# arnab39/equiadapt

Hardware: AMD Instinct MI355X
Metric: canonicalize+invert images/sec (224x224 C8) (higher is better)
Workload: dtype f32 (resampling / FFT / accumulation in fp32; the network's channel contraction as 2xfp16 split of every fp32 operand (within one fp32 ulp), 3 exact products, fp32 accumulate -- closer to fp64 than the fp32 matrix instruction, see step_ms_by_gemm_form); 1 GPU; configs[1]: 224x224x3 synthetic, C8, GroupEquivariantImageCanonicalization + ESCNNEquivariantNetwork in e2cnn's LAYER SHAPES (32 fields x 8 = 256 ch, k5, 3 layers, crop 0.8, resize 96) with this repository's own filter-bank parameterisation (bilinear-rotated banks; e2cnn's steerable basis is not restated -- e2cnn-trained weights enter via load_exported_dense), forward, then invert_canonicalization; batch_per_gpu=256, global_batch=256, parallelism=dp1 (no collective in the forward path)

## Files before the change

### equiadapt_amd/csrc/lift_fft.hip

```cpp
#include <cstdlib>

#include "eqa_common.hpp"

#ifndef EQA_LF_AUX
#define EQA_LF_AUX 2
#endif

namespace {

#include "fft_common.inc"

typedef float f32x4 __attribute__((ext_vector_type(4)));
typedef unsigned u32x4 __attribute__((ext_vector_type(4)));

#ifdef EQA_LF_CLOCK
__device__ unsigned long long g_lf_clock[32];
#define LF_CLOCK_BEGIN() const bool lfc_on = blockIdx.x == 0 && (threadIdx.x & 63) == 0 && (wave == 0 || wave == 1 || wave == 8); \
  unsigned long long lfc_t = __builtin_readcyclecounter(); unsigned long long lfc_s[16] = {0, 0, 0, 0, 0, 0, 0, 0, 0, 0, 0, 0, 0, 0, 0, 0}
#define LF_CLOCK(i) do { const unsigned long long n_ = __builtin_readcyclecounter(); lfc_s[i] += n_ - lfc_t; lfc_t = n_; } while (0)
#define LF_CLOCK_END() do { if (lfc_on) for (int i_ = 0; i_ < 8; ++i_) g_lf_clock[8 * (ROLE == kConv ? 0 : (wave == 1 ? 1 : 2)) + i_] = lfc_s[i_]; } while (0)
#else
#define LF_CLOCK_BEGIN() do { } while (0)
#define LF_CLOCK(i) do { } while (0)
#define LF_CLOCK_END() do { } while (0)
#endif

constexpr int kLfThreads = 768;
constexpr int kLfCh = 16;
constexpr int kLfSteps = 19;
constexpr int kLfQuadPitch = 196;
constexpr int kLfRowPitch = 784;
constexpr int kLfTileFloats = kFftN * kLfRowPitch;
constexpr int kLfSubRows = 16;
constexpr int kLfPatchRows = kLfSubRows + 4, kLfPatchPitch = 156;
constexpr int kLfPatchFloats = kLfPatchRows * kLfPatchPitch;
constexpr int kLfLdsFloats = kLfTileFloats + kLfPatchFloats;
constexpr int kLfStagers = 6 * 64;
constexpr int kLfPre = (kLfPatchFloats + kLfStagers - 1) / kLfStagers;

__device__ __forceinline__ void lf_slot(int n, int& ky, int& e, bool& spare) {
  spare = n == 75;
  const bool lo = n < 70;
  const int r = n % 14;
  ky = lo ? n / 14 : min(n - 70, 4);
  e = lo ? (r >> 1) + 8 * (r & 1) : 7;
}

struct LfItem {
  unsigned grp, m;
  int gy0, gx0;
  size_t img;
};

__device__ __forceinline__ LfItem lf_item(unsigned work, int ngrp, int TY, int TX) {
  LfItem it;
  it.grp = work % ngrp;
#ifdef EQA_LF_XCDGRP
  if (ngrp == 16) it.grp = 2 * (it.grp % 8) + it.grp / 8;
#endif
  it.m = work / ngrp;
  const unsigned tx = it.m % TX, ty = (it.m / TX) % TY;
  it.img = it.m / ((unsigned)TX * TY);
  it.gy0 = kFftO * (int)ty;
  it.gx0 = kFftO * (int)tx;
  return it;
}

enum { kConv = 0, kCols = 1, kRowp = 2 };

template <class F, int... Is>
__device__ __forceinline__ void lf_for_const(F&& f, std::integer_sequence<int, Is...>) {
  (f(std::integral_constant<int, Is>()), ...);
}

constexpr int kLpRowB = 53 * 8;
constexpr int kLpPlaneB = 8 * kLpRowB;
constexpr int kLpPatchB = 3 * kLpPlaneB;
constexpr int kLpLdsBytes = kLfTileFloats * 4 + kLpPatchB;
constexpr int kLhRowB = 52 * 8;
constexpr int kLhRing = 16;
constexpr int kLhPlaneB = kLhRing * kLhRowB;
constexpr int kLhPatchB = 2 * kLhPlaneB;
constexpr int kLhLdsBytes = kLfTileFloats * 4 + kLhPatchB;
constexpr int kLhSubRows = 12;
constexpr int kLhPre = 3;
typedef _Float16 lf_f16x8 __attribute__((ext_vector_type(8)));
typedef _Float16 lf_f16x4 __attribute__((ext_vector_type(4)));
typedef __bf16 lf_bf16x8 __attribute__((ext_vector_type(8)));
typedef __bf16 lf_bf16x4 __attribute__((ext_vector_type(4)));
__device__ __forceinline__ void lf_split3(float x, __bf16& p1, __bf16& p2, __bf16& p3) {
  p1 = (__bf16)x;
  const float r1 = x - (float)p1;
  p2 = (__bf16)r1;
  p3 = (__bf16)(r1 - (float)p2);
}

template <int ROLE, int FORM>
__device__ __forceinline__ void lift5_fft48_body(const float* __restrict__ x, const float* __restrict__ bank, const float* __restrict__ bias,
                                                 int relu, float* __restrict__ V, int H0, int W0, int C, int TY, int TX, size_t Mp,
                                                 unsigned nwork, unsigned v_bytes, unsigned x_bytes, unsigned bank_bytes,
                                                 float* __restrict__ dcmax, const float* __restrict__ xbound, int nxbound, float w_scale) {
  constexpr bool COLS = ROLE == kCols;
  constexpr bool PIECES = FORM == 3;
  constexpr bool H2 = FORM == 2;
  constexpr int NSUB = PIECES ? 12 : (H2 ? 4 : 3);
  constexpr int SUBROWS = kFftN / NSUB;
  constexpr int NGRP = 12 / NSUB;
  extern __shared__ float lds[];
  float* const tile = lds;
  float* const patch = lds + kLfTileFloats;
  const int tid = threadIdx.x;
  const int lane = tid & 63;
  const int wave = __builtin_amdgcn_readfirstlane(tid >> 6);
  const int j = lane & 15, q = lane >> 4;
  const int ngrp = C / kLfCh;
  const int H1 = H0 - 4, W1 = W0 - 4;
  const unsigned nblk = gridDim.x;
  const unsigned patch_b = (unsigned)(kLfTileFloats * 4);
  LF_CLOCK_BEGIN();

  const __amdgpu_buffer_rsrc_t xr = __builtin_amdgcn_make_buffer_rsrc(const_cast<float*>(x), 0, x_bytes, 0x00020000);
  float pre[COLS ? kLfPre : 1];
  auto prefetch = [&](const LfItem& it, int sub, bool live) {
    if constexpr (COLS) {
      int tq = tid;
      asm volatile("" : "+v"(tq));
#pragma unroll
      for (int i = 0; i < kLfPre; ++i) {
        const int idx = tq + kLfStagers * i;
        const int pr = idx / kLfPatchPitch, pc = idx - pr * kLfPatchPitch;
        const int gy = it.gy0 + kLfSubRows * sub + pr, gxc = it.gx0 * 3 + pc;
        const bool ok = live && idx < kLfPatchFloats && gy < H0 && gxc < W0 * 3;
        const unsigned off = ok ? (unsigned)(((it.img * H0 + gy) * (size_t)(W0 * 3) + gxc) * 4) : 0xfffffff0u;
        pre[i] = __builtin_bit_cast(float, __builtin_amdgcn_raw_buffer_load_b32(xr, off, 0, 0));
      }
    }
  };
  auto stage = [&]() {
    if constexpr (COLS) {
#pragma unroll
      for (int i = 0; i < kLfPre; ++i) {
        const int idx = tid + kLfStagers * i;
        if (idx < kLfPatchFloats) patch[idx] = pre[i];
      }
    }
  };

  float preg[COLS && PIECES ? 2 : 1][3];
  auto prefetch_grp = [&](const LfItem& it, int g, int which, bool live) {
    if constexpr (COLS && PIECES) {
      int tq = tid;
      asm volatile("" : "+v"(tq));
      const int pr = tq / 52, px = tq - pr * 52;
      const int gy = it.gy0 + 4 * g + pr, gx = it.gx0 + px;
      const bool ok = live && tq < 208 && gy < H0 && gx < W0;
      const unsigned off = ok ? (unsigned)((((it.img * H0 + gy) * (size_t)W0 + gx) * 3) * 4) : 0xfffffff0u;
#pragma unroll
      for (int c = 0; c < 3; ++c) preg[which][c] = __builtin_bit_cast(float, __builtin_amdgcn_raw_buffer_load_b32(xr, off, c * 4, 0));
    }
  };
  auto stage_grp = [&](int g, int which) {
    if constexpr (COLS && PIECES) {
      if (tid < 208) {
        const int pr = tid / 52, px = tid - pr * 52;
        __bf16 pc[3][3];
#pragma unroll
        for (int c = 0; c < 3; ++c) lf_split3(preg[which][c], pc[0][c], pc[1][c], pc[2][c]);
        char* dst = reinterpret_cast<char*>(lds) + patch_b + ((4 * g + pr) & 7) * kLpRowB + px * 8;
#pragma unroll
        for (int pl = 0; pl < 3; ++pl) {
          const lf_bf16x4 v = {pc[pl][0], pc[pl][1], pc[pl][2], (__bf16)0.0f};
          *reinterpret_cast<lf_bf16x4*>(dst + pl * kLpPlaneB) = v;
        }
      }
    }
  };

  float preh[(!COLS && H2) ? kLhPre : 1][3];
  float x_scale = 1.0f, out_scale = 1.0f;
  if constexpr (H2) {
    float mx = 0.0f;
    for (int t = lane; t < nxbound; t += 64) mx = fmaxf(mx, xbound[t]);
#pragma unroll
    for (int o = 32; o > 0; o >>= 1) mx = fmaxf(mx, __shfl_xor(mx, o));
    int ex = 0;
    if (mx > 0.0f && mx < 3.0e38f) (void)frexpf(mx, &ex);
    ex = __builtin_amdgcn_readfirstlane(min(max(14 - ex, -100), 100));
    x_scale = ldexpf(1.0f, ex);
    out_scale = ldexpf(1.0f, -ex) / w_scale;
  }
  int h_pr[(!COLS && H2) ? kLhPre : 1], h_px[(!COLS && H2) ? kLhPre : 1];
  if constexpr (!COLS && H2) {
#pragma unroll
    for (int i = 0; i < kLhPre; ++i) {
      const int idx = tid - 6 * 64 + kLfStagers * i;
      h_pr[i] = idx / 52;
      h_px[i] = idx - h_pr[i] * 52;
    }
  }
  auto prefetch_h = [&](const LfItem& it, int row0, int nrows, bool live) {
    if constexpr (!COLS && H2) {
#ifdef EQA_LF_H2_NOPREFETCH
      if (row0 >= 0) return;
#endif
#pragma unroll
      for (int i = 0; i < kLhPre; ++i) {
        const int pr = h_pr[i], px = h_px[i];
        const int gy = it.gy0 + row0 + pr, gx = it.gx0 + px;
        const bool ok = live && pr < nrows && gy < H0 && gx < W0;
        const unsigned off = ok ? (unsigned)((((it.img * H0 + gy) * (size_t)W0 + gx) * 3) * 4) : 0xfffffff0u;
#pragma unroll
        for (int c = 0; c < 3; ++c) preh[i][c] = __builtin_bit_cast(float, __builtin_amdgcn_raw_buffer_load_b32(xr, off, c * 4, 0));
      }
    }
  };
  auto stage_h = [&](int row0, int nrows) {
    if constexpr (!COLS && H2) {
#pragma unroll
      for (int i = 0; i < kLhPre; ++i) {
        asm volatile("" : "+v"(preh[i][0]), "+v"(preh[i][1]), "+v"(preh[i][2]));
        if (h_pr[i] < nrows) {
          const int pr = h_pr[i], px = h_px[i];
          _Float16 hi[3], lo[3];
#pragma unroll
          for (int c = 0; c < 3; ++c) {
            const float v = preh[i][c] * x_scale;
            hi[c] = (_Float16)v;
            lo[c] = (_Float16)(v - (float)hi[c]);
          }
          char* dst = reinterpret_cast<char*>(lds) + patch_b + ((row0 + pr) & (kLhRing - 1)) * kLhRowB + px * 8;
          const lf_f16x4 vh = {hi[0], hi[1], hi[2], (_Float16)0.0f}, vl = {lo[0], lo[1], lo[2], (_Float16)0.0f};
          *reinterpret_cast<lf_f16x4*>(dst) = vh;
          *reinterpret_cast<lf_f16x4*>(dst + kLhPlaneB) = vl;
        }
      }
    }
  };

  const int nr = (wave == 10 || wave == 11) ? 2 : 3;
  const int r0 = wave == 8 ? 0 : (wave == 9 ? 3 : (wave == 6 ? 6 : (wave == 10 ? 9 : (wave == 7 ? 11 : 14))));
  unsigned a_off[kLfSteps];
  float wreg[kLfSteps];
  f32x4 bias4;
  auto setup = [&](const LfItem& it) {
    const __amdgpu_buffer_rsrc_t br = __builtin_amdgcn_make_buffer_rsrc(const_cast<float*>(bank), 0, bank_bytes, 0x00020000);
    const unsigned wb = (unsigned)((it.grp * kLfCh + j) * 75 * 4);
#pragma unroll
    for (int t = 0; t < kLfSteps; ++t) {
      int ky, e;
      bool spare;
      lf_slot(4 * t + q, ky, e, spare);
      a_off[t] = patch_b + (unsigned)(((r0 + ky) * kLfPatchPitch + j * 3 + e) * 4);
      wreg[t] = __builtin_bit_cast(float, __builtin_amdgcn_raw_buffer_load_b32(br, spare ? 0xfffffff0u : wb + (unsigned)((ky * 15 + e) * 4), 0, 0));
    }
#pragma unroll
    for (int r = 0; r < 4; ++r) bias4[r] = bias ? bias[it.grp * kLfCh + 4 * q + r] : 0.0f;
    asm volatile("" : "+v"(bias4));
  };
#ifndef EQA_LF_AHEAD
#define EQA_LF_AHEAD 5
#endif
  constexpr int kAhead = EQA_LF_AHEAD;
  auto conv_rows = [&](const LfItem& it, int y0) {
    float b[3][kLfSteps], bq[2][3][kAhead];
    auto lds_at = [&](int t, int drow, int tx3) {
#ifdef EQA_LF_NOLDSREAD
      return __builtin_bit_cast(float, a_off[t] + (unsigned)(drow + tx3));
#else
      return reinterpret_cast<const float*>(reinterpret_cast<const char*>(lds) + a_off[t])[drow * kLfPatchPitch + tx3 * 48];
#endif
    };
#pragma unroll
    for (int t = 0; t < kAhead; ++t)
#pragma unroll
      for (int tx3 = 0; tx3 < 3; ++tx3) bq[0][tx3][t] = lds_at(t, 0, tx3);
#pragma unroll
    for (int r = 0; r < 3; ++r) {
      if (r < nr) {
        const int par = r & 1;
        const bool row_ok = it.gy0 + y0 + r < H1;
        f32x4 acc[3] = {bias4, bias4, bias4};
        __builtin_amdgcn_sched_barrier(0);
#pragma unroll
        for (int t = 0; t < kLfSteps; ++t) {
#pragma unroll
          for (int tx3 = 0; tx3 < 3; ++tx3)
#ifdef EQA_LF_NOMFMA
            acc[tx3][t & 3] += wreg[t] * (t < kAhead ? bq[par][tx3][t] : b[tx3][t]);
#else
            acc[tx3] = __builtin_amdgcn_mfma_f32_16x16x4f32(wreg[t], t < kAhead ? bq[par][tx3][t] : b[tx3][t], acc[tx3], 0, 0, 0);
#endif
          __builtin_amdgcn_sched_barrier(0);
          if (t + kAhead < kLfSteps) {
#pragma unroll
            for (int tx3 = 0; tx3 < 3; ++tx3) b[tx3][t + kAhead] = lds_at(t + kAhead, r, tx3);
          } else if (r + 1 < nr) {
#pragma unroll
            for (int tx3 = 0; tx3 < 3; ++tx3) bq[par ^ 1][tx3][t + kAhead - kLfSteps] = lds_at(t + kAhead - kLfSteps, r + 1, tx3);
          }
          __builtin_amdgcn_sched_barrier(0);
        }
#pragma unroll
        for (int tx3 = 0; tx3 < 3; ++tx3) {
          const bool ok = row_ok && it.gx0 + tx3 * 16 + j < W1;
          f32x4 v = acc[tx3];
#pragma unroll
          for (int k = 0; k < 4; ++k) {
            float u = relu ? fmaxf(v[k], 0.0f) : v[k];
            v[k] = ok ? u : 0.0f;
          }
          *reinterpret_cast<f32x4*>(tile + (y0 + r) * kLfRowPitch + q * kLfQuadPitch + (tx3 * 16 + j) * 4) = v;
        }
      }
    }
  };

  lf_bf16x8 wq[PIECES ? 4 : 1][PIECES ? 3 : 1];
  unsigned c_off[PIECES ? 4 : 1];
  int c_ky[PIECES ? 4 : 1];
  auto setup_p = [&](const LfItem& it) {
    if constexpr (PIECES) {
      const __amdgpu_buffer_rsrc_t br = __builtin_amdgcn_make_buffer_rsrc(const_cast<float*>(bank), 0, bank_bytes, 0x00020000);
#pragma unroll
      for (int sstep = 0; sstep < 4; ++sstep) {
        const int c = 4 * sstep + q;
        c_ky[sstep] = min(c / 3, 4);
        c_off[sstep] = (unsigned)((j + 2 * (c % 3)) * 8);
#pragma unroll
        for (int wp = 0; wp < 3; ++wp) {
          const unsigned off = (unsigned)((((it.grp * kLfCh + j) * 3 + wp) * 16 + c) * 16);
          wq[sstep][wp] = __builtin_bit_cast(lf_bf16x8, __builtin_amdgcn_raw_buffer_load_b128(br, off, 0, 0));
        }
      }
#pragma unroll
      for (int r = 0; r < 4; ++r) bias4[r] = bias ? bias[it.grp * kLfCh + 4 * q + r] : 0.0f;
      asm volatile("" : "+v"(bias4));
    }
  };
  auto conv_tiles_p = [&](const LfItem& it, int y, int tx0, auto NT) {
    constexpr int nt = decltype(NT)::value;
    if constexpr (PIECES) {
      const bool row_ok = it.gy0 + y < H1;
      unsigned addr[4];
#pragma unroll
      for (int sstep = 0; sstep < 4; ++sstep) addr[sstep] = patch_b + (unsigned)(((y + c_ky[sstep]) & 7) * kLpRowB) + c_off[sstep] + (unsigned)(tx0 * 16 * 8);
      f32x4 acc[3] = {bias4, bias4, bias4};
      lf_bf16x8 bp[2][3][3];
      auto read_step = [&](int sstep, int buf) {
#pragma unroll
        for (int t = 0; t < 3; ++t)
          if (t < nt)
#pragma unroll
            for (int pl = 0; pl < 3; ++pl)
#ifdef EQA_LF_NOLDSREAD
            {
              const f32x4 cv = {1.0f + (float)(addr[sstep] & 7), 0.5f + t, 0.25f + pl, 2.0f};
              bp[buf][t][pl] = __builtin_bit_cast(lf_bf16x8, cv);
            }
#else
            {
              typedef unsigned long long u64x2_t __attribute__((ext_vector_type(2)));
              const unsigned long long* pp = reinterpret_cast<const unsigned long long*>(reinterpret_cast<const char*>(lds) + addr[sstep] + t * 128 + pl * kLpPlaneB);
              const u64x2_t two = {pp[0], pp[1]};
              bp[buf][t][pl] = __builtin_bit_cast(lf_bf16x8, two);
            }
#endif
      };
      read_step(0, 0);
#pragma unroll
      for (int sstep = 0; sstep < 4; ++sstep) {
        const int buf = sstep & 1;
        if (sstep + 1 < 4) read_step(sstep + 1, buf ^ 1);
        __builtin_amdgcn_sched_barrier(0);
        constexpr int kW[6] = {2, 0, 1, 1, 0, 0}, kP[6] = {0, 2, 1, 0, 1, 0};
#pragma unroll
        for (int pr = 0; pr < 6; ++pr) {
#pragma unroll
          for (int t = 0; t < 3; ++t)
            if (t < nt) acc[t] = __builtin_amdgcn_mfma_f32_16x16x32_bf16(wq[sstep][kW[pr]], bp[buf][t][kP[pr]], acc[t], 0, 0, 0);
          __builtin_amdgcn_sched_barrier(0);
        }
      }
#pragma unroll
      for (int t = 0; t < 3; ++t) {
        if (t < nt) {
          const int tx3 = tx0 + t;
          const bool ok = row_ok && it.gx0 + tx3 * 16 + j < W1;
          f32x4 v = acc[t];
#pragma unroll
          for (int k = 0; k < 4; ++k) {
            float u = relu ? fmaxf(v[k], 0.0f) : v[k];
            v[k] = ok ? u : 0.0f;
          }
          *reinterpret_cast<f32x4*>(tile + y * kLfRowPitch + q * kLfQuadPitch + (tx3 * 16 + j) * 4) = v;
        }
      }
    }
  };

  lf_f16x8 wh[H2 ? 5 : 1][H2 ? 2 : 1];
  int h_off = 0;
  auto setup_h = [&](const LfItem& it) {
    if constexpr (H2) {
      const __amdgpu_buffer_rsrc_t br = __builtin_amdgcn_make_buffer_rsrc(const_cast<float*>(bank), 0, bank_bytes, 0x00020000);
#pragma unroll
      for (int ky = 0; ky < 5; ++ky)
#pragma unroll
        for (int wp = 0; wp < 2; ++wp) {
          const unsigned off = (unsigned)(((((it.grp * kLfCh + j) * 2 + wp) * 5 + ky) * 4 + q) * 16);
          wh[ky][wp] = __builtin_bit_cast(lf_f16x8, __builtin_amdgcn_raw_buffer_load_b128(br, off, 0, 0));
        }
#pragma unroll
      for (int r = 0; r < 4; ++r) bias4[r] = bias ? bias[it.grp * kLfCh + 4 * q + r] : 0.0f;
      asm volatile("" : "+v"(bias4));
    }
  };
  auto conv_col_h = [&](const LfItem& it, int y0, int t, auto NR) {
    if constexpr (H2) {
      constexpr int NROWS = decltype(NR)::value;
#ifdef EQA_LF_H2_NOCONV
      return;
#endif
      const int base = (int)patch_b + (j - 1 + 2 * min(q, 2)) * 8 + t * 128;
      lf_f16x8 win[7][2];
      auto read_row = [&](int k) {
        const int a = base + ((y0 + k) & (kLhRing - 1)) * kLhRowB;
#pragma unroll
        for (int pl = 0; pl < 2; ++pl) {
          typedef unsigned long long u64x2_t __attribute__((ext_vector_type(2)));
          const unsigned long long* pp = reinterpret_cast<const unsigned long long*>(reinterpret_cast<const char*>(lds) + a + pl * kLhPlaneB);
          const u64x2_t two = {pp[0], pp[1]};
          win[k % 7][pl] = __builtin_bit_cast(lf_f16x8, two);
        }
      };
#pragma unroll
      for (int k = 0; k < 6; ++k) read_row(k);
      const f32x4 zero = {0.0f, 0.0f, 0.0f, 0.0f};
      const bool col_ok = it.gx0 + t * 16 + j < W1;
      f32x4 acc[2];
      f32x4 ev = zero;
      auto epi = [&](int m, int rp) {
        const int y = y0 + rp;
        if (m == 0) ev = acc[rp & 1] * out_scale + bias4;
        else if (m == 1) { ev[0] = relu ? fmaxf(ev[0], 0.0f) : ev[0]; ev[1] = relu ? fmaxf(ev[1], 0.0f) : ev[1]; }
        else if (m == 2) { ev[2] = relu ? fmaxf(ev[2], 0.0f) : ev[2]; ev[3] = relu ? fmaxf(ev[3], 0.0f) : ev[3]; }
        else if (m == 3) {
          const bool ok = col_ok && it.gy0 + y < H1;
#pragma unroll
          for (int k = 0; k < 4; ++k) ev[k] = ok ? ev[k] : 0.0f;
        } else if (m == 4) {
          *reinterpret_cast<f32x4*>(tile + y * kLfRowPitch + q * kLfQuadPitch + (t * 16 + j) * 4) = ev;
        }
      };
#pragma unroll
      for (int r = 0; r < NROWS; ++r) {
#pragma unroll
        for (int m = 0; m < 15; ++m) {
          const int ky = m / 3, ch = m % 3;
          __builtin_amdgcn_sched_barrier(0);
          acc[r & 1] = __builtin_amdgcn_mfma_f32_16x16x32_f16(wh[ky][ch == 0 ? 1 : 0], win[(r + ky) % 7][ch == 1 ? 1 : 0], m == 0 ? zero : acc[r & 1], 0, 0, 0);
          if (r > 0 && m >= 2 && m < 7) epi(m - 2, r - 1);
          if (m == 9 && r + 2 < NROWS) read_row(r + 6);
        }
      }
      __builtin_amdgcn_sched_barrier(0);
#pragma unroll
      for (int m = 0; m < 5; ++m) epi(m, NROWS - 1);
    }
  };

  auto row_pass = [&](int y0) {
#ifdef EQA_LF_H2_NOROWP
    if (H2) return;
#endif
    float* const rowp = tile + (y0 + (lane >> 4)) * kLfRowPitch + ((lane & 15) >> 2) * kLfQuadPitch + (lane & 3);
    float re[kFftN], ore[kFftH], oim[kFftH];
#pragma unroll
    for (int xx = 0; xx < kFftN; ++xx) re[xx] = rowp[xx * 4];
    fft48_r2c(re, ore, oim);
#pragma unroll
    for (int k = 0; k < kFftH - 1; ++k) rowp[k * 4] = ore[k];
    rowp[24 * 4] = ore[24];
#pragma unroll
    for (int k = 1; k < kFftH - 1; ++k) rowp[(24 + k) * 4] = oim[k];
  };

  const int cw = COLS ? wave : 0;
  const int col_ci = lane >> 4, col_kxi = (lane >> 2) & 3, col_cq = lane & 3;
  const int kc_of0 = 8 * (cw >> 1) + 2 * (cw & 1) + (col_kxi >> 1);
  const int kc = kc_of0 + ((col_kxi & 1) ? 4 : 0);
  const bool odd = (col_kxi & 1) != 0;
  const bool has_packed = COLS && __builtin_amdgcn_readfirstlane((int)(cw == 0)) != 0;
  const bool pair_packed = COLS && kc_of0 == 0;
  const bool packed = COLS && kc == 0;
  const float* const colp = tile + col_cq * kLfQuadPitch + col_ci + kc * 4;
  const __amdgpu_buffer_rsrc_t vr = __builtin_amdgcn_make_buffer_rsrc(V, 0, v_bytes, 0x00020000);
  float cre[kFftN], cim[kFftN];
  unsigned pend_m = 0, pend_grp = 0;
  bool pending = false;
  float dc_seen = 0.0f;
  auto transpose4 = [&](float& r0_, float& r1_, float& r2_, float& r3_) {
    auto sw16 = [](float& a, float& b) { asm volatile("s_nop 1\n\tv_permlane16_swap_b32 %0, %1" : "+v"(a), "+v"(b)); };
    auto sw32 = [](float& a, float& b) { asm volatile("s_nop 1\n\tv_permlane32_swap_b32 %0, %1" : "+v"(a), "+v"(b)); };
    sw16(r0_, r1_);
    sw16(r2_, r3_);
    sw32(r0_, r2_);
    sw32(r1_, r3_);
  };
  auto swz4 = [](float v) { return __builtin_bit_cast(float, __builtin_amdgcn_ds_swizzle(__builtin_bit_cast(int, v), 0x101f)); };
  auto store_pair = [&](float* re, float* im, unsigned voff1, unsigned voff2, bool second) {
    transpose4(re[0], re[1], re[2], re[3]);
    transpose4(im[0], im[1], im[2], im[3]);
    f32x4 o1, o2;
#pragma unroll
    for (int r = 0; r < 4; ++r) {
      const float got = swz4(odd ? re[r] : im[r]);
      o1[r] = odd ? got : re[r];
      o2[r] = odd ? im[r] : got;
    }
    __builtin_amdgcn_raw_buffer_store_b128(__builtin_bit_cast(u32x4, o1), vr, voff1, 0, EQA_LF_AUX);
    if (second) __builtin_amdgcn_raw_buffer_store_b128(__builtin_bit_cast(u32x4, o2), vr, voff2, 0, EQA_LF_AUX);
  };
  auto col_work = [&](auto SUB) {
    constexpr int sub = decltype(SUB)::value;
    if (!pending) return;
#ifdef EQA_LF_H2_NOCOLS
    if (H2) return;
#endif
    const size_t rowb = Mp * 2 * (size_t)C * 4;
    const unsigned col = (unsigned)(((size_t)pend_m * 2 * C + pend_grp * 2 * kLfCh) * 4) + (unsigned)((odd ? 64 : 0) + 16 * col_cq);
    if (sub == 0) {
      float ore[kFftN], oim[kFftN];
      fft48(cre, cim, ore, oim);
#pragma unroll
      for (int ky = 0; ky < kFftN; ++ky) {
        cre[ky] = ore[ky];
        cim[ky] = oim[ky];
      }
      if (has_packed) {
        float p24re[28], p24im[28];
#pragma unroll
        for (int ky = 0; ky < kFftH; ++ky) {
          const int kn = (kFftN - ky) % kFftN;
          const float a = ore[ky], b = oim[ky], c2 = ore[kn], d = oim[kn];
          p24re[ky] = 0.5f * (b + d);
          p24im[ky] = 0.5f * (c2 - a);
          cre[ky] = packed ? 0.5f * (a + c2) : a;
          cim[ky] = packed ? 0.5f * (b - d) : b;
        }
        dc_seen = fmaxf(dc_seen, packed ? cre[0] : 0.0f);
#pragma unroll
        for (int ky = kFftH; ky < 28; ++ky) p24re[ky] = p24im[ky] = 0.0f;
#ifndef EQA_LF_NOSTORE
        const unsigned vb24 = (unsigned)((size_t)(kFftN * kFftInner + 1 + 2 * col_ci) * rowb) + col;
#pragma unroll
        for (int g = 0; g < 7; ++g) {
          const bool live = pair_packed && 4 * g + col_ci < kFftH;
          store_pair(&p24re[4 * g], &p24im[4 * g], live ? vb24 + (unsigned)g * (unsigned)(8 * rowb) : 0xfffffff0u, 0xfffffff0u, false);
        }
#endif
      }
    }
#ifndef EQA_LF_NOSTORE
    const unsigned f1 = pair_packed ? (unsigned)(kFftN * kFftInner + 2 * col_ci) : (unsigned)(kFftInner * col_ci + kc_of0 - 1);
    const unsigned vb1 = (unsigned)((size_t)f1 * rowb) + col, vs1 = (unsigned)((pair_packed ? 8 : 4 * kFftInner) * rowb);
    const unsigned vb2 = (unsigned)((size_t)(kFftInner * col_ci + kc_of0 + 3) * rowb) + col, vs2 = (unsigned)(4 * kFftInner * rowb);
#pragma unroll
    for (int g = NGRP * sub; g < NGRP * sub + NGRP; ++g) {
      const bool live1 = !pair_packed || 4 * g + col_ci < kFftH;
      store_pair(&cre[4 * g], &cim[4 * g], live1 ? vb1 + (unsigned)g * vs1 : 0xfffffff0u, vb2 + (unsigned)g * vs2, true);
    }
#endif
  };

  unsigned cur_grp = 0xffffffffu;
  unsigned v = blockIdx.x;
  if constexpr (PIECES) {
    if (COLS && tid < 24) *reinterpret_cast<unsigned long long*>(reinterpret_cast<char*>(lds) + patch_b + tid * kLpRowB + 52 * 8) = 0ull;
    const LfItem f = lf_item(v < nwork ? v : 0, ngrp, TY, TX);
    prefetch_grp(f, 0, 0, v < nwork);
    prefetch_grp(f, 1, 1, v < nwork);
    stage_grp(0, 0);
    stage_grp(1, 1);
  } else if constexpr (H2) {
    if (tid == 0) *reinterpret_cast<unsigned long long*>(reinterpret_cast<char*>(lds) + patch_b - 8) = 0ull;
    prefetch_h(lf_item(v < nwork ? v : 0, ngrp, TY, TX), 0, kLhRing, v < nwork);
    stage_h(0, kLhRing);
    __syncthreads();
  } else {
    if (v < nwork) prefetch(lf_item(v, ngrp, TY, TX), 0, true);
    stage();
    __syncthreads();
  }
  for (;; v += nblk) {
    const bool live = v < nwork;
    if (!live && !pending) break;
    const LfItem it = lf_item(live ? v : 0, ngrp, TY, TX);
    const unsigned vn = v + nblk;
    const bool next_live = live && vn < nwork;
    const LfItem nx = lf_item(next_live ? vn : 0, ngrp, TY, TX);
    if constexpr (!COLS) {
#pragma unroll 1
      for (int sub = 0; sub < NSUB; ++sub) {
        if (PIECES || sub > 0) __syncthreads();
        LF_CLOCK(0);
        if constexpr (H2) {
          if (sub < NSUB - 1) prefetch_h(it, kLhSubRows * sub + kLhRing, kLhSubRows, live);
          else prefetch_h(nx, 0, kLhRing, next_live);
          LF_CLOCK(1);
        }
        if (live) {
          if (sub == 0 && it.grp != cur_grp) {
            if constexpr (PIECES) setup_p(it);
            else if constexpr (H2) { if constexpr (ROLE == kConv) setup_h(it); }
            else setup(it);
            cur_grp = it.grp;
          }
          if constexpr (H2) {
            if constexpr (ROLE == kConv) {
              conv_col_h(it, kLhSubRows * sub, wave - 8, std::integral_constant<int, kLhSubRows>());
            } else {
              if (sub > 0) row_pass(kLhSubRows * (sub - 1) + 4 * (wave == 11 ? 2 : wave - 6));
            }
          } else if constexpr (PIECES) {
            const int y = SUBROWS * sub + (wave == 8 ? 0 : (wave == 9 ? 1 : ((wave == 6 || wave == 10) ? 2 : 3)));
            const int tx0 = (wave == 10 || wave == 11) ? 2 : 0;
            if (wave == 8 || wave == 9) conv_tiles_p(it, y, tx0, std::integral_constant<int, 3>());
            else if (wave == 10 || wave == 11) conv_tiles_p(it, y, tx0, std::integral_constant<int, 1>());
            else conv_tiles_p(it, y, tx0, std::integral_constant<int, 2>());
          } else {
            conv_rows(it, kLfSubRows * sub + r0);
            if (sub > 0 && (wave == 8 || wave == 9)) row_pass(8 * (sub - 1) + 4 * (wave - 8));
          }
        }
        LF_CLOCK(2);
        __syncthreads();
        LF_CLOCK(3);
        if constexpr (H2) {
          if (sub < NSUB - 1) stage_h(kLhSubRows * sub + kLhRing, kLhSubRows);
          else stage_h(0, kLhRing);
        }
      }
    } else {
      auto subphase = [&](auto SUB) {
        constexpr int sub = decltype(SUB)::value;
        if constexpr (FORM == 0) {
          if (sub > 0) stage();
        }
        if (PIECES || sub > 0) __syncthreads();
        LF_CLOCK(0);
        if constexpr (H2) {
        } else if constexpr (PIECES) {
          if (sub < NSUB - 1) {
            prefetch_grp(it, sub + 2, 0, live);
          } else {
            prefetch_grp(nx, 0, 0, next_live);
            prefetch_grp(nx, 1, 1, next_live);
          }
        } else {
          if (sub < NSUB - 1) prefetch(it, sub + 1, live);
          else prefetch(nx, 0, next_live);
        }
        LF_CLOCK(1);
        col_work(SUB);
        LF_CLOCK(2);
        __syncthreads();
        LF_CLOCK(3);
        if constexpr (PIECES) {
          if (sub < NSUB - 1) {
            stage_grp(sub + 2, 0);
          } else {
            stage_grp(0, 0);
            stage_grp(1, 1);
          }
        }
      };
      lf_for_const(subphase, std::make_integer_sequence<int, NSUB>());
      if constexpr (FORM == 0) stage();
    }
    if constexpr (PIECES) {
      if (live) row_pass(4 * wave);
    } else if constexpr (H2) {
      if constexpr (ROLE == kRowp) {
        if (live) row_pass(36 + 4 * (wave == 11 ? 2 : wave - 6));
      }
    } else {
      if (live && wave < 8) row_pass(16 + 4 * wave);
    }
    LF_CLOCK(4);
    __syncthreads();
    LF_CLOCK(5);
    constexpr int kEarly = PIECES ? kFftN : (H2 ? kLhSubRows : kLfSubRows);
    if constexpr (COLS) {
      if (live) {
#pragma unroll
        for (int y = 0; y < kEarly; ++y) {
          cre[y] = colp[y * kLfRowPitch];
          cim[y] = colp[y * kLfRowPitch + 24 * 4];
        }
      }
    }
    LF_CLOCK(6);
    __syncthreads();
    LF_CLOCK(7);
    if constexpr (COLS && !PIECES) {
      if (live) {
#pragma unroll
        for (int y = kEarly; y < kFftN; ++y) {
          cre[y] = colp[y * kLfRowPitch];
          cim[y] = colp[y * kLfRowPitch + 24 * 4];
        }
      }
    }
    pend_m = it.m;
    pend_grp = it.grp;
    pending = live;
  }
  if constexpr (COLS) {
    if (dcmax != nullptr && has_packed) {
      float m = dc_seen;
#pragma unroll
      for (int o = 32; o > 0; o >>= 1) m = fmaxf(m, __shfl_xor(m, o));
      if (lane == 0) dcmax[blockIdx.x] = m;
      if (blockIdx.x == 0) {
        for (unsigned t = nblk + lane; t < (unsigned)EQA_LIFT5_DCMAX_SLOTS; t += 64) dcmax[t] = 0.0f;
      }
    }
  }
  LF_CLOCK_END();
}

__global__ __launch_bounds__(kLfThreads) void lift5_fft48_fused_kernel(const float* __restrict__ x, const float* __restrict__ bank,
                                                                        const float* __restrict__ bias, int relu, float* __restrict__ V,
                                                                        int H0, int W0, int C, int TY, int TX, size_t Mp, unsigned nwork,
                                                                        unsigned v_bytes, unsigned x_bytes, unsigned bank_bytes,
                                                                        float* __restrict__ dcmax) {
  if (threadIdx.x < 6 * 64) lift5_fft48_body<kCols, 0>(x, bank, bias, relu, V, H0, W0, C, TY, TX, Mp, nwork, v_bytes, x_bytes, bank_bytes, dcmax, nullptr, 0, 1.0f);
  else lift5_fft48_body<kConv, 0>(x, bank, bias, relu, V, H0, W0, C, TY, TX, Mp, nwork, v_bytes, x_bytes, bank_bytes, dcmax, nullptr, 0, 1.0f);
}

__global__ __launch_bounds__(kLfThreads) void lift5_fft48_fused_pieces_kernel(const float* __restrict__ x, const float* __restrict__ bank,
                                                                               const float* __restrict__ bias, int relu, float* __restrict__ V,
                                                                               int H0, int W0, int C, int TY, int TX, size_t Mp, unsigned nwork,
                                                                               unsigned v_bytes, unsigned x_bytes, unsigned bank_bytes,
                                                                               float* __restrict__ dcmax) {
  if (threadIdx.x < 6 * 64) lift5_fft48_body<kCols, 3>(x, bank, bias, relu, V, H0, W0, C, TY, TX, Mp, nwork, v_bytes, x_bytes, bank_bytes, dcmax, nullptr, 0, 1.0f);
  else lift5_fft48_body<kConv, 3>(x, bank, bias, relu, V, H0, W0, C, TY, TX, Mp, nwork, v_bytes, x_bytes, bank_bytes, dcmax, nullptr, 0, 1.0f);
}

__global__ __launch_bounds__(kLfThreads) void lift5_fft48_fused_h2_kernel(const float* __restrict__ x, const float* __restrict__ bank,
                                                                           const float* __restrict__ bias, int relu, float* __restrict__ V,
                                                                           int H0, int W0, int C, int TY, int TX, size_t Mp, unsigned nwork,
                                                                           unsigned v_bytes, unsigned x_bytes, unsigned bank_bytes,
                                                                           float* __restrict__ dcmax, const float* __restrict__ xbound,
                                                                           int nxbound, float w_scale) {
  const int w = __builtin_amdgcn_readfirstlane((int)(threadIdx.x >> 6));
  if (w < 6) lift5_fft48_body<kCols, 2>(x, bank, bias, relu, V, H0, W0, C, TY, TX, Mp, nwork, v_bytes, x_bytes, bank_bytes, dcmax, xbound, nxbound, w_scale);
  else if (w >= 8 && w <= 10) lift5_fft48_body<kConv, 2>(x, bank, bias, relu, V, H0, W0, C, TY, TX, Mp, nwork, v_bytes, x_bytes, bank_bytes, dcmax, xbound, nxbound, w_scale);
  else lift5_fft48_body<kRowp, 2>(x, bank, bias, relu, V, H0, W0, C, TY, TX, Mp, nwork, v_bytes, x_bytes, bank_bytes, dcmax, xbound, nxbound, w_scale);
}

__global__ __launch_bounds__(256) void absmax_slots_kernel(const float* __restrict__ x, size_t n, float* __restrict__ out) {
  float m = 0.0f;
  const size_t n4 = n / 4;
  for (size_t i = (size_t)blockIdx.x * 256 + threadIdx.x; i < n4; i += (size_t)gridDim.x * 256) {
    const f32x4 v = reinterpret_cast<const f32x4*>(x)[i];
    m = fmaxf(fmaxf(m, fmaxf(fabsf(v[0]), fabsf(v[1]))), fmaxf(fabsf(v[2]), fabsf(v[3])));
  }
  if (blockIdx.x == 0 && threadIdx.x < (n & 3)) m = fmaxf(m, fabsf(x[n4 * 4 + threadIdx.x]));
  __shared__ float red[4];
#pragma unroll
  for (int o = 32; o > 0; o >>= 1) m = fmaxf(m, __shfl_xor(m, o));
  if ((threadIdx.x & 63) == 0) red[threadIdx.x >> 6] = m;
  __syncthreads();
  if (threadIdx.x == 0) out[blockIdx.x] = fmaxf(fmaxf(red[0], red[1]), fmaxf(red[2], red[3]));
}

}

extern "C" {

#ifdef EQA_LF_CLOCK
int eqa_debug_lf_clock(unsigned long long* out) { return hipMemcpyFromSymbol(out, HIP_SYMBOL(g_lf_clock), sizeof(g_lf_clock)) == hipSuccess ? 0 : -1; }
#endif

int eqa_lift5_fft48k5_input_supported(int Cin, int KH, int KW, int Cout) {
  return (Cin == 3 && KH == 5 && KW == 5 && Cout > 0 && Cout % kLfCh == 0) ? 1 : 0;
}

static int lift_fft_launch(const float* x, const void* bank, size_t bank_bytes, const float* bias, int relu, float* V, int nimg, int H0, int W0,
                           int Cout, void* stream, bool pieces, float* dcmax = nullptr, const float* xbound = nullptr, int nxbound = 0,
                           float w_scale = 0.0f) {
  if (!x || !bank || !V || nimg < 0 || H0 < 5 || W0 < 5 || Cout <= 0) return EQA_ERR_INVALID_ARG;
  if (Cout % kLfCh != 0) return EQA_ERR_UNSUPPORTED;
  if (nimg == 0) return EQA_OK;
  const int H1 = H0 - 4, W1 = W0 - 4;
  const int TY = (int)eqa_fft48k5_tiles(H1), TX = (int)eqa_fft48k5_tiles(W1);
  if (TY <= 0 || TX <= 0) return EQA_ERR_UNSUPPORTED;
  const size_t M = (size_t)nimg * TY * TX;
  const size_t nwork = M * (Cout / kLfCh);
  const size_t vb = (size_t)kFftF * fft_pitch(M) * 2 * Cout * 4;
  const size_t xb = (size_t)nimg * H0 * W0 * 3 * 4;
  if (nwork > 0x7fffffffULL || vb > 0xffffff00ULL || xb > 0xffffff00ULL || bank_bytes > 0xffffff00ULL) return EQA_ERR_UNSUPPORTED;
  const bool h2 = xbound != nullptr;
  const void* kern = h2 ? (const void*)lift5_fft48_fused_h2_kernel : pieces ? (const void*)lift5_fft48_fused_pieces_kernel : (const void*)lift5_fft48_fused_kernel;
  const int lds_bytes = h2 ? kLhLdsBytes : pieces ? kLpLdsBytes : kLfLdsFloats * 4;
  if (!allow_dynamic_lds(kern, lds_bytes)) return EQA_ERR_UNSUPPORTED;
  const unsigned ngrp = (unsigned)(Cout / kLfCh);
  unsigned nblk = 256;
  if (ngrp <= 256) nblk = (256 / ngrp) * ngrp;
  if ((size_t)nblk > nwork) nblk = (unsigned)nwork;
  if (h2)
    hipLaunchKernelGGL(lift5_fft48_fused_h2_kernel, dim3(nblk), dim3(kLfThreads), lds_bytes, (hipStream_t)stream, x, (const float*)bank, bias,
                       relu, V, H0, W0, Cout, TY, TX, fft_pitch(M), (unsigned)nwork, (unsigned)vb, (unsigned)xb, (unsigned)bank_bytes, dcmax,
                       xbound, nxbound, w_scale);
  else if (pieces)
    hipLaunchKernelGGL(lift5_fft48_fused_pieces_kernel, dim3(nblk), dim3(kLfThreads), lds_bytes, (hipStream_t)stream, x, (const float*)bank, bias,
                       relu, V, H0, W0, Cout, TY, TX, fft_pitch(M), (unsigned)nwork, (unsigned)vb, (unsigned)xb, (unsigned)bank_bytes, dcmax);
  else
    hipLaunchKernelGGL(lift5_fft48_fused_kernel, dim3(nblk), dim3(kLfThreads), lds_bytes, (hipStream_t)stream, x, (const float*)bank, bias,
                       relu, V, H0, W0, Cout, TY, TX, fft_pitch(M), (unsigned)nwork, (unsigned)vb, (unsigned)xb, (unsigned)bank_bytes, dcmax);
  return launch_status();
}

int eqa_lift5_fft48k5_input(const float* x, const float* bank, const float* bias, int relu, float* V, int nimg, int H0, int W0, int Cout,
                            void* stream) {
  return lift_fft_launch(x, bank, (size_t)(Cout > 0 ? Cout : 0) * 75 * 4, bias, relu, V, nimg, H0, W0, Cout, stream, false);
}

int eqa_lift5_fft48k5_input_dcmax(const float* x, const float* bank, const float* bias, int relu, float* V, float* dcmax, int nimg, int H0,
                                  int W0, int Cout, void* stream) {
  if (!dcmax) return EQA_ERR_INVALID_ARG;
  if (!relu) return EQA_ERR_UNSUPPORTED;
  if (nimg == 0) return hipMemsetAsync(dcmax, 0, EQA_LIFT5_DCMAX_SLOTS * sizeof(float), (hipStream_t)stream) == hipSuccess ? EQA_OK : EQA_ERR_LAUNCH;
  return lift_fft_launch(x, bank, (size_t)(Cout > 0 ? Cout : 0) * 75 * 4, bias, relu, V, nimg, H0, W0, Cout, stream, false, dcmax);
}

int64_t eqa_lift5_pieces_f16_bytes(int Cout) { return Cout > 0 ? (int64_t)Cout * 2 * 5 * 4 * 8 * 2 : 0; }

int eqa_absmax_slots(const float* x, int64_t n, float* slots, void* stream) {
  if (n < 0 || !slots || (n > 0 && !x)) return EQA_ERR_INVALID_ARG;
  if (((uintptr_t)x & 15) != 0) return EQA_ERR_UNSUPPORTED;
  hipLaunchKernelGGL(absmax_slots_kernel, dim3(EQA_LIFT5_DCMAX_SLOTS), dim3(256), 0, (hipStream_t)stream, x, (size_t)n, slots);
  return launch_status();
}

int eqa_lift5_fft48k5_input_f16x2(const float* x, const void* wpieces, float w_scale, const float* xbound, int nxbound, const float* bias,
                                  int relu, float* V, float* dcmax, int nimg, int H0, int W0, int Cout, void* stream) {
  if (!xbound || nxbound <= 0 || !(w_scale > 0.0f)) return EQA_ERR_INVALID_ARG;
  int ex = 0;
  if (frexpf(w_scale, &ex) != 0.5f) return EQA_ERR_INVALID_ARG;
  if (dcmax && !relu) return EQA_ERR_UNSUPPORTED;
  if (nimg == 0 && dcmax) return hipMemsetAsync(dcmax, 0, EQA_LIFT5_DCMAX_SLOTS * sizeof(float), (hipStream_t)stream) == hipSuccess ? EQA_OK : EQA_ERR_LAUNCH;
  return lift_fft_launch(x, wpieces, (size_t)eqa_lift5_pieces_f16_bytes(Cout), bias, relu, V, nimg, H0, W0, Cout, stream, false, dcmax, xbound,
                         nxbound, w_scale);
}

int64_t eqa_lift5_pieces_bytes(int Cout) { return Cout > 0 ? (int64_t)Cout * 3 * 16 * 8 * 2 : 0; }

int eqa_lift5_fft48k5_input_bf16x3(const float* x, const void* wpieces, const float* bias, int relu, float* V, int nimg, int H0, int W0,
                                   int Cout, void* stream) {
  return lift_fft_launch(x, wpieces, (size_t)eqa_lift5_pieces_bytes(Cout), bias, relu, V, nimg, H0, W0, Cout, stream, true);
}

}
```

Baseline: 67780 images/s.

## Rebalance H2 fused lift kernel: four conv waves and redistributed row-pass work

The fused H2 lift kernel now sends waves 8-11 to the MFMA convolution role instead of 8-10. Each conv wave covers 9 rows, with two waves crossing between column tiles mid-sweep by reloading their LDS row window. The row-FFT pass work is redistributed through a per-wave table (lf_h2_rows) so some kCols waves also take row passes. The aim is to balance the conv and row-FFT critical paths within a sub-block. In exchange it adds irregular tile crossings, extra LDS reloads and more complex scheduling. The clock instrumentation is extended to more waves and to record hardware IDs.

```diff
diff --git a/equiadapt_amd/csrc/lift_fft.hip b/equiadapt_amd/csrc/lift_fft.hip
--- a/equiadapt_amd/csrc/lift_fft.hip
+++ b/equiadapt_amd/csrc/lift_fft.hip
@@ -14,11 +14,13 @@
 typedef unsigned u32x4 __attribute__((ext_vector_type(4)));
 
 #ifdef EQA_LF_CLOCK
-__device__ unsigned long long g_lf_clock[32];
-#define LF_CLOCK_BEGIN() const bool lfc_on = blockIdx.x == 0 && (threadIdx.x & 63) == 0 && (wave == 0 || wave == 1 || wave == 8); \
+__device__ unsigned long long g_lf_clock[64];
+__device__ __forceinline__ int lf_clock_slot(int wave) { return wave == 8 ? 0 : wave == 1 ? 1 : wave == 0 ? 2 : wave == 6 ? 3 : wave == 11 ? 4 : -1; }
+#define LF_CLOCK_BEGIN() const bool lfc_on = blockIdx.x == 0 && (threadIdx.x & 63) == 0 && lf_clock_slot(wave) >= 0; \
+  if (blockIdx.x == 0 && (threadIdx.x & 63) == 0) { unsigned hw_; asm volatile("s_getreg_b32 %0, hwreg(HW_REG_HW_ID)" : "=s"(hw_)); g_lf_clock[40 + wave] = hw_; } \
   unsigned long long lfc_t = __builtin_readcyclecounter(); unsigned long long lfc_s[16] = {0, 0, 0, 0, 0, 0, 0, 0, 0, 0, 0, 0, 0, 0, 0, 0}
 #define LF_CLOCK(i) do { const unsigned long long n_ = __builtin_readcyclecounter(); lfc_s[i] += n_ - lfc_t; lfc_t = n_; } while (0)
-#define LF_CLOCK_END() do { if (lfc_on) for (int i_ = 0; i_ < 8; ++i_) g_lf_clock[8 * (ROLE == kConv ? 0 : (wave == 1 ? 1 : 2)) + i_] = lfc_s[i_]; } while (0)
+#define LF_CLOCK_END() do { if (lfc_on) for (int i_ = 0; i_ < 8; ++i_) g_lf_clock[8 * lf_clock_slot(wave) + i_] = lfc_s[i_]; } while (0)
 #else
 #define LF_CLOCK_BEGIN() do { } while (0)
 #define LF_CLOCK(i) do { } while (0)
@@ -67,6 +69,18 @@
 }
 
 enum { kConv = 0, kCols = 1, kRowp = 2 };
+
+#ifdef EQA_LF_H2_ROWS_IN_SUB
+__device__ __forceinline__ int lf_h2_rows(int wave, int s) {
+  if (s < 4) return wave == 6 ? (1 | ((s & 1) ? 4 : 0)) : (wave == 7 ? (2 | ((s & 1) ? 0 : 4)) : 0);
+  return wave == 6 ? 36 : wave == 7 ? 40 : wave == 4 ? 44 : -1;
+}
+#else
+__device__ __forceinline__ int lf_h2_rows(int wave, int s) {
+  if (s < 4) return wave == 6 ? 1 : (wave == 7 ? 2 : 0);
+  return wave == 6 ? 36 : wave == 7 ? 40 : wave == 0 ? 8 : wave == 4 ? 20 : wave == 1 ? 32 : wave == 5 ? 44 : -1;
+}
+#endif
 
 template <class F, int... Is>
 __device__ __forceinline__ void lf_for_const(F&& f, std::integer_sequence<int, Is...>) {
@@ -415,16 +429,17 @@
       asm volatile("" : "+v"(bias4));
     }
   };
-  auto conv_col_h = [&](const LfItem& it, int y0, int t, auto NR) {
+  auto conv_col_h = [&](const LfItem& it, int y0, int t0, int y1, int t1, bool cross) {
     if constexpr (H2) {
-      constexpr int NROWS = decltype(NR)::value;
+      constexpr int NROWS = 9, SW = 3;
 #ifdef EQA_LF_H2_NOCONV
       return;
 #endif
-      const int base = (int)patch_b + (j - 1 + 2 * min(q, 2)) * 8 + t * 128;
+      const int base0 = (int)patch_b + (j - 1 + 2 * min(q, 2)) * 8 + t0 * 128;
+      const int base1 = base0 + (t1 - t0) * 128;
       lf_f16x8 win[7][2];
-      auto read_row = [&](int k) {
-        const int a = base + ((y0 + k) & (kLhRing - 1)) * kLhRowB;
+      auto read_row = [&](int k, bool NEW) {
+        const int a = (NEW ? base1 + ((y1 + k - SW) & (kLhRing - 1)) * kLhRowB : base0 + ((y0 + k) & (kLhRing - 1)) * kLhRowB);
 #pragma unroll
         for (int pl = 0; pl < 2; ++pl) {
           typedef unsigned long long u64x2_t __attribute__((ext_vector_type(2)));
@@ -434,18 +449,19 @@
         }
       };
 #pragma unroll
-      for (int k = 0; k < 6; ++k) read_row(k);
+      for (int k = 0; k < 6; ++k) read_row(k, false);
       const f32x4 zero = {0.0f, 0.0f, 0.0f, 0.0f};
-      const bool col_ok = it.gx0 + t * 16 + j < W1;
+      const bool col_ok0 = it.gx0 + t0 * 16 + j < W1, col_ok1 = it.gx0 + t1 * 16 + j < W1;
       f32x4 acc[2];
       f32x4 ev = zero;
       auto epi = [&](int m, int rp) {
-        const int y = y0 + rp;
+        const int y = rp < SW ? y0 + rp : y1 + rp - SW;
+        const int t = rp < SW ? t0 : t1;
         if (m == 0) ev = acc[rp & 1] * out_scale + bias4;
         else if (m == 1) { ev[0] = relu ? fmaxf(ev[0], 0.0f) : ev[0]; ev[1] = relu ? fmaxf(ev[1], 0.0f) : ev[1]; }
         else if (m == 2) { ev[2] = relu ? fmaxf(ev[2], 0.0f) : ev[2]; ev[3] = relu ? fmaxf(ev[3], 0.0f) : ev[3]; }
         else if (m == 3) {
-          const bool ok = col_ok && it.gy0 + y < H1;
+          const bool ok = (rp < SW ? col_ok0 : col_ok1) && it.gy0 + y < H1;
 #pragma unroll
           for (int k = 0; k < 4; ++k) ev[k] = ok ? ev[k] : 0.0f;
         } else if (m == 4) {
@@ -454,13 +470,18 @@
       };
 #pragma unroll
       for (int r = 0; r < NROWS; ++r) {
+        if (r == SW && cross) {
+          __builtin_amdgcn_sched_barrier(0);
+#pragma unroll
+          for (int k = SW; k < SW + 4; ++k) read_row(k, true);
+        }
 #pragma unroll
         for (int m = 0; m < 15; ++m) {
           const int ky = m / 3, ch = m % 3;
           __builtin_amdgcn_sched_barrier(0);
           acc[r & 1] = __builtin_amdgcn_mfma_f32_16x16x32_f16(wh[ky][ch == 0 ? 1 : 0], win[(r + ky) % 7][ch == 1 ? 1 : 0], m == 0 ? zero : acc[r & 1], 0, 0, 0);
           if (r > 0 && m >= 2 && m < 7) epi(m - 2, r - 1);
-          if (m == 9 && r + 2 < NROWS) read_row(r + 6);
+          if (m == 9 && r + 2 < NROWS) read_row(r + 6, r + 6 >= SW + 4);
         }
       }
       __builtin_amdgcn_sched_barrier(0);
@@ -618,9 +639,17 @@
           }
           if constexpr (H2) {
             if constexpr (ROLE == kConv) {
-              conv_col_h(it, kLhSubRows * sub, wave - 8, std::integral_constant<int, kLhSubRows>());
+              const int y = kLhSubRows * sub;
+              const bool cross = wave == 9 || wave == 10;
+              const int ya = y + (wave == 8 || wave == 10 ? 0 : (wave == 9 ? 9 : 3)), ta = wave == 8 || wave == 9 ? 0 : 2;
+              conv_col_h(it, ya, ta, cross ? y + (wave == 9 ? 0 : 6) : ya + 3, cross ? 1 : ta, cross);
             } else {
-              if (sub > 0) row_pass(kLhSubRows * (sub - 1) + 4 * (wave == 11 ? 2 : wave - 6));
+              if (sub > 0) {
+                const int a = lf_h2_rows(wave, sub);
+#pragma unroll 1
+                for (int k = 0; k < 3; ++k)
+                  if (a & (1 << k)) row_pass(kLhSubRows * (sub - 1) + 4 * k);
+              }
             }
           } else if constexpr (PIECES) {
             const int y = SUBROWS * sub + (wave == 8 ? 0 : (wave == 9 ? 1 : ((wave == 6 || wave == 10) ? 2 : 3)));
@@ -681,8 +710,9 @@
     if constexpr (PIECES) {
       if (live) row_pass(4 * wave);
     } else if constexpr (H2) {
-      if constexpr (ROLE == kRowp) {
-        if (live) row_pass(36 + 4 * (wave == 11 ? 2 : wave - 6));
+      if constexpr (ROLE != kConv) {
+        const int a = lf_h2_rows(wave, NSUB);
+        if (live && a >= 0) row_pass(a);
       }
     } else {
       if (live && wave < 8) row_pass(16 + 4 * wave);
@@ -756,7 +786,7 @@
                                                                            int nxbound, float w_scale) {
   const int w = __builtin_amdgcn_readfirstlane((int)(threadIdx.x >> 6));
   if (w < 6) lift5_fft48_body<kCols, 2>(x, bank, bias, relu, V, H0, W0, C, TY, TX, Mp, nwork, v_bytes, x_bytes, bank_bytes, dcmax, xbound, nxbound, w_scale);
-  else if (w >= 8 && w <= 10) lift5_fft48_body<kConv, 2>(x, bank, bias, relu, V, H0, W0, C, TY, TX, Mp, nwork, v_bytes, x_bytes, bank_bytes, dcmax, xbound, nxbound, w_scale);
+  else if (w >= 8) lift5_fft48_body<kConv, 2>(x, bank, bias, relu, V, H0, W0, C, TY, TX, Mp, nwork, v_bytes, x_bytes, bank_bytes, dcmax, xbound, nxbound, w_scale);
   else lift5_fft48_body<kRowp, 2>(x, bank, bias, relu, V, H0, W0, C, TY, TX, Mp, nwork, v_bytes, x_bytes, bank_bytes, dcmax, xbound, nxbound, w_scale);
 }
 
```

After: 69550 images/s (median of 6 runs). 2.6% higher.
